# LIS-TU-Berlin/SVN-ICP

Measured on AMD Instinct MI355X. Metric: scan-pair registrations/sec at N particles x M source pts, 1/2/4/8 GPU, higher is better.
Workload: dtype f64; 1 GPU; C3: 128 particles SVN-ICP, 131072-pt source vs 262144-pt target, K=100, I=20, max_dist=1.0, lr=1.0, SVNFullGrad=False, correspondence=fast, early stop off; synthetic 64-beam scans (seed 20250718); particles=128, target_points=262144, knn_count=100, parallelism=single GPU

## Files before the change

### svn-icp_amd/csrc/api.hip

```cpp
#include "../../include/svnicp_hip.h"

#include <cmath>
#include <algorithm>
#include <cstdio>
#include <cstdlib>
#include <cstring>
#include <string>
#include <vector>

#include "device_buffer.hpp"
#include "information_solve.hpp"
#include "kernels.hpp"
#include "pose_prior.hpp"
#include "stage_a_host.hpp"
#include "stage_b_host.hpp"

using namespace svnicp;
using namespace svnicp_host;

namespace {

struct CloudState {
  DevBuf<double> src, tgt;
  bool src_set = false, tgt_set = false;
// ... 354 lines not shown
    HIPCHK(c, hipEventSynchronize(c->st.ev_init));
  }
  std::memcpy(c->st.h_init.p, init, (size_t)P * 48);
  HIPCHK(c, hipMemcpyAsync(c->st.init_pose.p, c->st.h_init.p, (size_t)P * 48, hipMemcpyHostToDevice, c->stream));
  HIPCHK(c, hipEventRecord(c->st.ev_init, c->stream));
  c->st.init_in_flight = true;
  c->st.host_stats_valid = false;
  const bool first = !c->run.particles_set || P != c->P;
  if (P != c->P) c->sc.have = false;
  c->sc.of_result = false;
  if (first && c->shard.row_world > 1) { c->shard.row_world = 1; c->shard.row_rank = 0; c->shard.B_total = 0; }
  c->P = P;
  if (!c->shard.set || first) { c->shard.p_lo = 0; c->shard.p_hi = P; c->shard.set = false; }
  HIPCHK(c, launch_init_particles(c->st.init_pose.p, P, c->pose0, c->prm.mode, c->st.R.p, c->st.t.p, c->st.Rtot.p, c->st.pose_out.p,
                                  (first || c->prm.mode == SVNICP_MODE_SVN) ? 1 : 0, c->st.eul.p, c->stream));
  c->run.particles_set = true;
  return SVNICP_OK;
}

int svnicp_set_initial_mean(svnicp_ctx* c, const double R0[9], const double t0[3]) {
  CTX_CHECK(c);
  if (!R0 || !t0) return fail(c, SVNICP_ERR_INVALID, "svnicp_set_initial_mean: null argument");
  std::memcpy(c->pose0.R0, R0, 9 * sizeof(double));
  std::memcpy(c->pose0.t0, t0, 3 * sizeof(double));
  c->run.have_candidates = false;
  return SVNICP_OK;
}

int svnicp_set_k(svnicp_ctx* c, int k) {
  CTX_CHECK(c);
  if (k < 1) return fail(c, SVNICP_ERR_INVALID, "svnicp_set_k: k >= 1 required");
  c->K = k;
  c->run.have_candidates = false;
  return SVNICP_OK;
}

int svnicp_set_max_dist(svnicp_ctx* c, double md) {
  CTX_CHECK(c);
  c->prm.max_dist = md;
  return SVNICP_OK;
}

int svnicp_set_option(svnicp_ctx* c, const char* name, const char* value) {
  CTX_CHECK(c);
  if (!name || !value) return fail(c, SVNICP_ERR_INVALID, "svnicp_set_option: null argument");
  const std::string k(name), v(value);
  Tuning& t = c->tune;
  auto num = [&](int lo, int hi, int* out) { char* end = nullptr; const long x = strtol(v.c_str(), &end, 10);
                                             if (end == v.c_str() || *end || x < lo || x > hi) return false; *out = (int)x; return true; };
  bool ok = true;
  if (k == "knn") { if (v == "auto") t.knn = {}; else if (v == "v1") t.knn = {false, KnnKernel::Stream}; else if (v == "v2") t.knn = {false, KnnKernel::SeededScan};
                    else if (v == "brute") t.knn = {false, KnnKernel::Brute}; else if (v == "tiles") t.knn = {false, KnnKernel::Tiles}; else ok = false; }
  else if (k == "knn_prefilter") { if (v == "mfma") t.knn_prefilter_mfma = 1; else if (v == "valu") t.knn_prefilter_mfma = 0; else ok = false; }
  else if (k == "fallback_sliced_max") ok = num(-1, 1 << 20, &t.fallback_sliced_max);
  else if (k == "accum") { if (v == "f64") t.accum = 0; else if (v == "valu") t.accum = 1; else if (v == "split") t.accum = 3; else ok = false; }
  else if (k == "update") { if (v == "auto") t.update_fused = 0; else if (v == "fused") t.update_fused = 1; else ok = false; }
  else if (k == "fused_update_max_p") ok = num(1, 700, &t.fused_update_max_p);
  else if (k == "wgpcu") { int x = 0, y = 0; ok = sscanf(v.c_str(), "%d,%d", &x, &y) == 2 && x >= 0 && x <= 64 && y >= 0 && y <= 16; if (ok) { t.wgpcu_search = x; t.wgpcu_accum = y; } }
  else if (k == "tp") ok = num(0, 1 << 16, &t.tp);
  else if (k == "debug") ok = num(0, 1, &t.debug);
  else if (k == "scan_split") ok = num(0, 16, &t.scan_split);
  else if (k == "group_stride") ok = num(0, 1 << 30, &t.group_stride);
  else if (k == "accum_min_steps") ok = num(0, 1 << 20, &t.accum_min_steps);
  else if (k == "brute_qb") { ok = num(0, 6, &t.brute_qb); }
  else if (k == "single") { if (v == "fused") t.single_fused = 1; else if (v == "split") t.single_fused = 0; else ok = false; }
  else if (k == "chain") { if (v == "auto") { t.small_chain = 1; t.persistent = 0; } else if (v == "persistent") { t.small_chain = 1; t.persistent = 1; }
                           else if (v == "general") { t.small_chain = 0; t.persistent = 0; } else ok = false; }
  else if (k == "median") { if (v == "auto") t.median_inline = -1; else if (v == "stream") t.median_inline = 0; else if (v == "inline") t.median_inline = 1; else ok = false; }
  else if (k == "sort") { if (v == "joint") t.sort_joint = 1; else if (v == "separate") t.sort_joint = 0; else ok = false; }
  else if (k == "sort_kernel") { if (v == "radix") t.sort_merge = 0; else if (v == "merge") t.sort_merge = 1; else ok = false; }
  else if (k == "table") { if (v == "select") t.table_select = 1; else if (v == "gather") t.table_select = 0; else ok = false; }
  else if (k == "correspondence") { if (v == "fast") t.full_corr = 0; else if (v == "full") t.full_corr = 1; else ok = false; }
  else return fail(c, SVNICP_ERR_INVALID, "svnicp_set_option: unknown option '" + k + "'");
  if (!ok) return fail(c, SVNICP_ERR_INVALID, "svnicp_set_option: bad value '" + v + "' for option '" + k + "'");
  c->run.have_candidates = false;
  c->sa.held = TargetLayout::None;
  if (c->run.began) c->st.step = plan_step(registration_facts(c, c->pl.on, c->pr.on), c->tune, c->sb.plan);
  return SVNICP_OK;
}

int svnicp_set_shard(svnicp_ctx* c, int p_lo, int p_hi) {
  CTX_CHECK(c);
  if (!c->run.particles_set || p_lo < 0 || p_hi > c->P || p_lo > p_hi)
    return fail(c, SVNICP_ERR_INVALID, "svnicp_set_shard: need 0 <= p_lo <= p_hi <= P after svnicp_set_particles");
  c->shard.p_lo = p_lo; c->shard.p_hi = p_hi; c->shard.set = true;
  return SVNICP_OK;
}

int svnicp_set_row_shard(svnicp_ctx* c, int row_rank, int row_world, int64_t total_source_points) {
  CTX_CHECK(c);
  if (!c->run.particles_set || row_world < 1 || row_rank < 0 || row_rank >= row_world || (row_world > 1 && total_source_points < 1))
    return fail(c, SVNICP_ERR_INVALID, "svnicp_set_row_shard: need 0 <= row_rank < row_world and the whole scan's point count, after svnicp_set_particles");
  if (bind(c)) return SVNICP_ERR_HIP;
  c->shard.row_rank = row_rank; c->shard.row_world = row_world;
  c->shard.B_total = row_world > 1 ? total_source_points : 0;
  if (row_world > 1) {
    HIPCHK(c, c->shard.rank_sums.ensure((size_t)row_world * c->P * kNSums));
    HIPCHK(c, hipMemsetAsync(c->shard.rank_sums.p, 0, (size_t)row_world * c->P * kNSums * sizeof(double), c->stream));
  }
  return SVNICP_OK;
}

void* svnicp_rank_sums_devptr(svnicp_ctx* c) { return (c && c->shard.row_world > 1) ? (void*)c->shard.rank_sums.p : nullptr; }

static bool normal_pass_due(const svnicp_ctx* c) {
  return c->pl.on && !c->pl.supplied && !(c->pl.estimated && c->pl.est_k == c->pl.normal_k);
// ... 1043 lines not shown
```

### svn-icp_amd/csrc/kernels.hpp

```cpp
#pragma once
#include "device_math.hpp"
#include "registration_plan.hpp"
#include "stage_a_plan.hpp"

namespace svnicp {

struct KnnArgs {
  const double* src;
  Pose0 pose;
  const double *tx, *ty, *tz;
  const int32_t* torig;
  int64_t M, Mp;
  int64_t b_lo, b_hi;
  int K, S;
  double* pool_d;
  int32_t* pool_i;
  int32_t* out_idx;
  double* out_d2;
  const int32_t* qlist;
  const int* qlist_count;
  int list_grid;
  int list_qw;
  int slices, slice_max_queries, merge_n;
  double* sl_d;
  int32_t* sl_i;
  const double* qthr;
};
hipError_t launch_knn_merge_slices(const KnnArgs& a, hipStream_t st);

struct KnnBruteArgs {
  const double* src;
  Pose0 pose;
  const double* tgt;
  int64_t M;
  int64_t b_lo, b_hi;
  int K;
  int32_t* out_idx;
  double* out_d2;
  unsigned long long* phase_cycles;
};
int knn_brute_queries_per_block(int64_t n, int num_cus);
hipError_t launch_knn_brute(const KnnBruteArgs& a, int num_cus, int queries_per_block, hipStream_t st);

struct KnnScanArgs {
  const double* src;
  Pose0 pose;
  const double *tx, *ty, *tz;
  const float *txf, *tyf, *tzf;
  const int32_t* torig;
  const unsigned long long* emax_bits;
  int64_t M, Mp, Ms;
  int64_t b_lo, b_hi;
  int K, S2, seed_rank;
  int32_t* pool;
  int32_t* out_idx;
  double* out_d2;
  int32_t* fail_list;
  int* fail_count;
};
hipError_t launch_targets_soa2(const double* tgt, int64_t M, int64_t Mp, double* tx, double* ty, double* tz,
                               float* txf, float* tyf, float* tzf, int32_t* torig, unsigned long long* emax_bits,
                               hipStream_t st);
hipError_t launch_knn_scan(const KnnScanArgs& a, hipStream_t st);
hipError_t launch_knn_topk(const KnnArgs& a, hipStream_t st);

struct KnnTilesArgs {
  const double* src;
  Pose0 pose;
  const int32_t* qorder;
  const double *tx, *ty, *tz;
  const float *txf, *tyf, *tzf;
  const int32_t* torig;
  const float* tile_box;
  const unsigned long long* emax_bits;
  const float4* tile_a;
  const float4* tile_o;
  int prefilter_mfma;
  int64_t M, Mp;
  int n_tiles;
  int64_t b_lo, b_hi;
  int K, S2;
  int32_t* pool;
  int32_t* arena;
  int32_t* chunk_tab;
  int arena_cap;
  int64_t tab_rows;
  int scan_split;
  unsigned int group_stride;
  int32_t* out_idx;
  double* out_d2;
  const double* tgt;
  float4* tbl_a;
  double* tbl_anchor;
  float* tbl_cmax;
  int32_t* fail_list;
  int* fail_count;
  int32_t* stat_n;
  unsigned long long* phase_cycles;
  void* qrec;
  double* fail_tau;
};
hipError_t launch_knn_tiles(const KnnTilesArgs& a, hipStream_t st);
hipError_t launch_candidate_dist2(const double* src, const Pose0& pose, const double* tgt, int64_t M, const int32_t* idx, int64_t B, int K,
                                  double* d2, hipStream_t st);
size_t sort_temp_bytes(size_t n, int key_bits);
hipError_t launch_bbox(const double* pts, int64_t n, unsigned long long* bbox, bool cleared, hipStream_t st);
hipError_t launch_morton_order(const double* pts, int64_t i0, int64_t n, int transform, const Pose0& pose,
                               const unsigned long long* bbox, unsigned int* keys_a, unsigned int* keys_b,
                               int32_t* vals_a, int32_t* order, void* temp, size_t temp_bytes, bool rocprim_sort, int32_t* fill_ff,
                               size_t fill_words, hipStream_t st);
hipError_t launch_morton_order_joint(const double* tgt, int64_t M, const double* qsrc, int64_t n, const Pose0& pose,
                                     const unsigned long long* bbox, unsigned int* keys_a, unsigned int* keys_b,
                                     int32_t* vals_a, int32_t* order, void* temp, size_t temp_bytes, bool rocprim_sort, int32_t* fill_ff,
                                     size_t fill_words, hipStream_t st);
hipError_t launch_targets_sorted(const double* tgt, int64_t M, int64_t Mp, const int32_t* order, double* tx, double* ty,
                                 double* tz, float* txf, float* tyf, float* tzf, int32_t* torig, float* tile_box,
                                 unsigned long long* emax_bits, bool emax_cleared, float4* tile_a, float4* tile_o, hipStream_t st);

struct AccumArgs {
  const double* src;
  const double* table;
  const float4* tablef;
  const float4* tablea;
  const float* cmax;
  int* ambig_count;
  const double* Rtot;
  int64_t B;
  int K, RS;
  int p_lo, p_hi;
  int TP;
// ... 200 lines not shown
```

### svn-icp_amd/csrc/knn_tiles.hip

```cpp
#include "kernels.hpp"
#include "stein_split_device.hpp"

namespace svnicp {

namespace {

constexpr int T = 8;
constexpr int STEP = kWave * T;
constexpr int QW = 64;
constexpr int WAVES = 4;
constexpr int QCAP = 1024;
constexpr int SL = 512;
constexpr int NSQ = 4;
constexpr int MAX_TILES = 8192;
constexpr int QB = 16;
constexpr double kU = 5.9604644775390625e-08;
constexpr float kEpsTile = 56.0f * 5.9604644775390625e-08f;

struct alignas(16) QF { float x, y, z, thr; };
struct alignas(16) QD { double x, y, z, tau; };

__device__ __forceinline__ void wave_sync() {
  __builtin_amdgcn_fence(__ATOMIC_ACQ_REL, "wavefront");
  __builtin_amdgcn_wave_barrier();
// ... 206 lines not shown
    return;
  }
  if (m <= 2 * kWave) {
    for (int e = m + lane; e < 2 * kWave + 8; e += kWave) { sd[e] = __builtin_huge_val(); si[e] = 0x7fffffff; }
    wave_sync();
    const int e0 = lane, e1 = lane + kWave;
    const double d0 = e0 < m ? sd[e0] : 0.0, d1 = e1 < m ? sd[e1] : 0.0;
    const int i0 = e0 < m ? si[e0] : 0, i1 = e1 < m ? si[e1] : 0;
    const P3 c0 = target_row(a, a.tbl_a && e0 < m, i0), c1 = target_row(a, a.tbl_a && e1 < m, i1);
    int* flag = si + 2 * kWave + 8;
    flag[lane] = 0; flag[lane + kWave] = 0;
    int r0 = 0, r1 = 0;
    for (int j0 = 0; j0 < m; j0 += 8) {
      double dj[8];
#pragma unroll
      for (int u = 0; u < 8; ++u) dj[u] = sd[j0 + u];
#pragma unroll
      for (int u = 0; u < 8; ++u) {
        r0 += dj[u] < d0 ? 1 : 0;
        r1 += dj[u] < d1 ? 1 : 0;
      }
    }
    wave_sync();
    if (e0 < m) atomicAdd(&flag[r0], 1);
    if (e1 < m) atomicAdd(&flag[r1], 1);
    wave_sync();
    if (__ballot((e0 < m && flag[r0] > 1) || (e1 < m && flag[r1] > 1))) {
      for (int j = 0; j < m; ++j) {
        const double dj = sd[j];
        const int ij = si[j];
        r0 += (dj == d0 && ij < i0) ? 1 : 0;
        r1 += (dj == d1 && ij < i1) ? 1 : 0;
      }
    }
    if (e0 < m && r0 < K) { a.out_idx[b * K + r0] = i0; if (a.out_d2) a.out_d2[b * K + r0] = d0; }
    if (e1 < m && r1 < K) { a.out_idx[b * K + r1] = i1; if (a.out_d2) a.out_d2[b * K + r1] = d1; }
    if (a.tbl_a) write_table_row(a, b, e0 < m ? r0 : -1, c0, e1 < m ? r1 : -1, c1, sd, lane);
    wave_sync();
  } else {
    int S = 256;
    while (S < m) S <<= 1;
    for (int e = m + lane; e < S; e += kWave) { sd[e] = __builtin_huge_val(); si[e] = 0x7fffffff; }
    wave_sync();
    bitonic_sort(sd, si, S, lane);
    for (int e = lane; e < K; e += kWave) { a.out_idx[b * K + e] = si[e]; if (a.out_d2) a.out_d2[b * K + e] = sd[e]; }
    if (a.tbl_a) {
      const int e1 = lane + kWave;
      write_table_row(a, b, lane, target_row(a, lane < K, si[lane]), e1, target_row(a, e1 < K, e1 < K ? si[e1] : 0), sd, lane);
    }
    wave_sync();
  }
}

__global__ __launch_bounds__(256) void k_knn_seed(KnnTilesArgs a) {
  extern __shared__ __align__(16) unsigned char smem[];
  const int lane = threadIdx.x & (kWave - 1);
  const int wave = __builtin_amdgcn_readfirstlane(threadIdx.x >> 6);
  const int K = a.K, n_tiles = a.n_tiles;
  constexpr size_t kShared = sizeof(QD) * QW + sizeof(QF) * QW + 4 * sizeof(int) * QW + sizeof(unsigned int) * (MAX_TILES / 32);
  constexpr size_t kScratch = sizeof(float2) * QB * kWave + 512;
  static_assert(QB * WAVES == QW, "one batch per wave");
  QD* qd = reinterpret_cast<QD*>(smem);
  QF* qf = reinterpret_cast<QF*>(smem + sizeof(QD) * QW);
  int* cnt = reinterpret_cast<int*>(smem + (sizeof(QD) + sizeof(QF)) * QW);
  int* qb = cnt + QW;
  float* thrb = reinterpret_cast<float*>(qb + QW);
  int* spare = reinterpret_cast<int*>(thrb + QW);
  unsigned int* tbits = reinterpret_cast<unsigned int*>(spare + QW);
  unsigned char* scratch = smem + kShared + kScratch * wave;
  float2* lm = reinterpret_cast<float2*>(scratch);

  const unsigned int grp = blockIdx.x;
  const int64_t q0 = a.b_lo + (int64_t)grp * QW;
  const int nq = (a.b_hi - q0) < QW ? (int)(a.b_hi - q0) : QW;
  const double Et = __longlong_as_double((long long)*a.emax_bits);

  unsigned long long tphase = a.phase_cycles ? __builtin_readcyclecounter() : 0ull;
  unsigned long long pacc[8] = {0, 0, 0, 0, 0, 0, 0, 0};
  auto phase_mark = [&](int i) {
    if (!a.phase_cycles) return;
    const unsigned long long now = __builtin_readcyclecounter();
    pacc[i] += now - tphase;
    tphase = now;
  };
  float wlo0 = 0.f, wlo1 = 0.f, wlo2 = 0.f, whi0 = 0.f, whi1 = 0.f, whi2 = 0.f;
  const int nwords = (n_tiles + 31) >> 5;
  if (wave == 0) {
    const bool act = lane < nq;
    const int64_t b = act ? (int64_t)a.qorder[q0 - a.b_lo + lane] : 0;
    QD s; s.x = s.y = s.z = 0.0; s.tau = 0.0;
    if (act) {
      stage_a_query(a.pose, a.src[3 * b], a.src[3 * b + 1], a.src[3 * b + 2], &s.x, &s.y, &s.z);
    }
    qd[lane] = s;
    QF f; f.x = (float)s.x; f.y = (float)s.y; f.z = (float)s.z; f.thr = -1.0f;
    qf[lane] = f;
    cnt[lane] = 0; qb[lane] = (int)b; thrb[lane] = -1.0f;
    const float inf = __builtin_huge_valf();
    wlo0 = act ? f32_floor(s.x) : inf; wlo1 = act ? f32_floor(s.y) : inf; wlo2 = act ? f32_floor(s.z) : inf;
    whi0 = act ? f32_ceil(s.x) : -inf; whi1 = act ? f32_ceil(s.y) : -inf; whi2 = act ? f32_ceil(s.z) : -inf;
    for (int off = 32; off > 0; off >>= 1) {
      wlo0 = __builtin_fminf(wlo0, __shfl_xor(wlo0, off, kWave)); whi0 = __builtin_fmaxf(whi0, __shfl_xor(whi0, off, kWave));
      wlo1 = __builtin_fminf(wlo1, __shfl_xor(wlo1, off, kWave)); whi1 = __builtin_fmaxf(whi1, __shfl_xor(whi1, off, kWave));
      wlo2 = __builtin_fminf(wlo2, __shfl_xor(wlo2, off, kWave)); whi2 = __builtin_fmaxf(whi2, __shfl_xor(whi2, off, kWave));
    }
  }
  wave_sync();
  const float* bx_lo0 = a.tile_box, *bx_lo1 = a.tile_box + n_tiles, *bx_lo2 = a.tile_box + 2 * (size_t)n_tiles;
  const float* bx_hi0 = a.tile_box + 3 * (size_t)n_tiles, *bx_hi1 = a.tile_box + 4 * (size_t)n_tiles,
             * bx_hi2 = a.tile_box + 5 * (size_t)n_tiles;

  {
    if (wave == 0) {
      for (int e = lane; e < nwords; e += kWave) tbits[e] = 0u;
      wave_sync();
      const float px = qf[lane].x, py = qf[lane].y, pz = qf[lane].z;
      unsigned long long best[NSQ];
#pragma unroll
      for (int i = 0; i < NSQ; ++i) best[i] = ~0ull;
      float4* boxs = reinterpret_cast<float4*>(scratch);
      const int n_groups = (n_tiles + kWave - 1) / kWave;
      unsigned int gkey[2] = {0xffffffffu, 0xffffffffu};
      for (int g = 0; g < n_groups; ++g) {
        const int tl = g * kWave + lane;
        const float inf = __builtin_huge_valf();
        float lo0 = inf, lo1 = inf, lo2 = inf, hi0 = -inf, hi1 = -inf, hi2 = -inf;
        if (tl < n_tiles) { lo0 = bx_lo0[tl]; lo1 = bx_lo1[tl]; lo2 = bx_lo2[tl]; hi0 = bx_hi0[tl]; hi1 = bx_hi1[tl]; hi2 = bx_hi2[tl]; }
        for (int off = 32; off > 0; off >>= 1) {
          lo0 = __builtin_fminf(lo0, __shfl_xor(lo0, off, kWave)); hi0 = __builtin_fmaxf(hi0, __shfl_xor(hi0, off, kWave));
          lo1 = __builtin_fminf(lo1, __shfl_xor(lo1, off, kWave)); hi1 = __builtin_fmaxf(hi1, __shfl_xor(hi1, off, kWave));
          lo2 = __builtin_fminf(lo2, __shfl_xor(lo2, off, kWave)); hi2 = __builtin_fmaxf(hi2, __shfl_xor(hi2, off, kWave));
        }
        const float glb = box_lb2(wlo0, wlo1, wlo2, whi0, whi1, whi2, lo0, lo1, lo2, hi0, hi1, hi2);
        const unsigned int key = (glb < inf) ? ((__float_as_uint(glb) & ~127u) | (unsigned int)g) : 0xffffffffu;
        if (lane == (g & (kWave - 1))) gkey[g >> 6] = key;
      }
      for (;;) {
        unsigned int kmin = gkey[0] < gkey[1] ? gkey[0] : gkey[1];
        for (int off = 32; off > 0; off >>= 1) { const unsigned int o = __shfl_xor(kmin, off, kWave); kmin = o < kmin ? o : kmin; }
        if (kmin == 0xffffffffu) break;
        float w4 = -__builtin_huge_valf();
        if (lane < nq) w4 = best[NSQ - 1] == ~0ull ? __builtin_huge_valf() : __uint_as_float((unsigned int)(best[NSQ - 1] >> 32));
        for (int off = 32; off > 0; off >>= 1) w4 = __builtin_fmaxf(w4, __shfl_xor(w4, off, kWave));
        if (__uint_as_float(kmin & ~127u) > w4) break;
        const int gsel = (int)(kmin & 127u);
        if (lane == (gsel & (kWave - 1))) gkey[gsel >> 6] = 0xffffffffu;
        const int t0 = gsel * kWave;
        const int tl = t0 + lane;
        if (tl < n_tiles) {
          boxs[2 * lane] = make_float4(bx_lo0[tl], bx_lo1[tl], bx_lo2[tl], bx_hi0[tl]);
          boxs[2 * lane + 1] = make_float4(bx_hi1[tl], bx_hi2[tl], 0.f, 0.f);
        }
        wave_sync();
        const int cntt = (n_tiles - t0) < kWave ? (n_tiles - t0) : kWave;
#pragma unroll 4
        for (int i = 0; i < cntt; ++i) {
          const float4 b0 = boxs[2 * i], b1 = boxs[2 * i + 1];
          const float l0 = b0.x, l1 = b0.y, l2 = b0.z, h0 = b0.w, h1 = b1.x, h2 = b1.y;
          const int tile = t0 + i;
          const float lb = box_lb2(px, py, pz, px, py, pz, l0, l1, l2, h0, h1, h2);
          const float c0 = px - 0.5f * (l0 + h0), c1 = py - 0.5f * (l1 + h1), c2 = pz - 0.5f * (l2 + h2);
          const float score = lb + 1e-3f * (c0 * c0 + c1 * c1 + c2 * c2);
          unsigned long long key = (score < __builtin_huge_valf()) ? (((unsigned long long)__float_as_uint(score) << 32) | (unsigned int)tile) : ~0ull;
#pragma unroll
          for (int u = 0; u < NSQ; ++u) {
            const unsigned long long lo = key < best[u] ? key : best[u];
            key = key < best[u] ? best[u] : key;
            best[u] = lo;
          }
        }
        wave_sync();
      }
      if (lane < nq) {
#pragma unroll
        for (int i = 0; i < NSQ; ++i)
          if (best[i] != ~0ull) { const unsigned int t = (unsigned int)(best[i] & 0xffffffffull); atomicOr(&tbits[t >> 5], 1u << (t & 31)); }
      }
    }
    phase_mark(0);
    __syncthreads();
    phase_mark(3);
    const int qb0 = wave * QB;
    if (qb0 < nq) {
      const int nb = (nq - qb0) < QB ? (nq - qb0) : QB;
      for (int e = lane; e < QB * kWave; e += kWave) lm[e] = make_float2(__builtin_huge_valf(), __builtin_huge_valf());
      wave_sync();
      for (int wd = 0; wd < nwords; ++wd) {
        unsigned int bits = __builtin_amdgcn_readfirstlane(tbits[wd]);
        while (bits) {
          const int tile = (wd << 5) + (int)__builtin_ctz(bits);
          bits &= bits - 1;
          if (a.phase_cycles) pacc[4] += 1;
          const int64_t tb = (int64_t)tile * STEP;
          float x[T], y[T], z[T];
#pragma unroll
          for (int t = 0; t < T; ++t) { x[t] = a.txf[tb + t * kWave + lane]; y[t] = a.tyf[tb + t * kWave + lane]; z[t] = a.tzf[tb + t * kWave + lane]; }
          for (int q = 0; q < nb; ++q) {
            const float4 cur = *reinterpret_cast<const float4*>(&qf[qb0 + q]);
            float2 m = lm[q * kWave + lane];
#pragma unroll
            for (int t = 0; t < T; ++t) {
              const float dx = cur.x - x[t], dy = cur.y - y[t], dz = cur.z - z[t];
              float d = __builtin_fmaf(dz, dz, __builtin_fmaf(dy, dy, dx * dx));
              d = __builtin_fminf(d, __builtin_huge_valf());
              m.y = __builtin_amdgcn_fmed3f(m.x, m.y, d);
              m.x = __builtin_fminf(m.x, d);
            }
            lm[q * kWave + lane] = m;
          }
        }
      }
      wave_sync();
      phase_mark(5);
      for (int q = 0; q < nb; ++q) {
        const float2 m = lm[q * kWave + lane];
        const unsigned int kx = __float_as_uint(m.x), ky = __float_as_uint(m.y);
        unsigned int kth = 0u;
        for (int bit = 30; bit >= 0; --bit) {
          const unsigned int t_try = kth | ((1u << bit) - 1u);
          const int c = __popcll(__ballot(kx <= t_try)) + __popcll(__ballot(ky <= t_try));
          if (c < K) kth |= 1u << bit;
        }
        if (lane == 0) spare[qb0 + q] = (int)kth;
      }
      phase_mark(6);
    }
    phase_mark(1);
    __syncthreads();
    phase_mark(3);
    if (wave == 0 && lane < nq) {
      const double tv = (double)__uint_as_float((unsigned int)spare[lane]);
      const double E = fmax(Et, fmax(fabs(qd[lane].x), fmax(fabs(qd[lane].y), fabs(qd[lane].z))));
      double tau = __builtin_huge_val();
      if (tv < (double)__builtin_huge_valf()) {
        const double r = sqrt(tv) * (1.0 + 1e-6) + 4.0 * kU * E;
        tau = (r * r) * (1.0 + 1e-12);
      }
      qd[lane].tau = tau;
      const float thr = filter_threshold(tau, E);
      qf[lane].thr = thr;
      float tb = __builtin_huge_valf();
      if (thr < __builtin_huge_valf()) {
        const double rb = sqrt((double)thr) + 2.0 * kU * E;
        tb = f32_round_up((rb * rb) * (1.0 + 1e-6));
      }
      thrb[lane] = tb;
    }
    wave_sync();
  }

  if (wave == 0 && lane < nq) {
    QRec rec;
    rec.x = qd[lane].x; rec.y = qd[lane].y; rec.z = qd[lane].z; rec.tau = qd[lane].tau;
    rec.cnt = 0; rec.row = qb[lane]; rec.thr = qf[lane].thr; rec.tb = thrb[lane];
    reinterpret_cast<QRec*>(a.qrec)[q0 + lane] = rec;
  }
  phase_mark(1);
  if (a.phase_cycles && lane == 0) {
#pragma unroll
    for (int i = 0; i < 5; ++i) atomicAdd(&a.phase_cycles[i], pacc[i]);
    unsigned long long* pw = a.phase_cycles + 8 + 8 * ((size_t)grp * WAVES + wave);
#pragma unroll
    for (int i = 0; i < 7; ++i) pw[i] = pacc[i];
  }
}

template <int SW, bool MF>
__global__ __launch_bounds__(64 * SW) __attribute__((amdgpu_waves_per_eu(4, 4))) void k_knn_scan_tiles(KnnTilesArgs a) {
  __shared__ __align__(16) QF s_qf[QW];
  __shared__ int s_cnt[QW];
  __shared__ int s_ticket;
  __shared__ __align__(16) int2 s_queue[SW][QCAP];
  __shared__ __align__(16) float4 s_lb[MF ? SW : 1][QW];
  __shared__ float s_lth[MF ? SW : 1][QW];
  __shared__ int s_lq[MF ? SW : 1][QW];
  const int lane = threadIdx.x & (kWave - 1);
  const int wave = __builtin_amdgcn_readfirstlane(threadIdx.x >> 6);
  const int S2 = a.S2, n_tiles = a.n_tiles;
  int2* queue = s_queue[wave];
  const unsigned int ngrp = gridDim.x;
  const unsigned int grp = (unsigned int)(((unsigned long long)blockIdx.x * a.group_stride) % ngrp);
  const int64_t q0 = a.b_lo + (int64_t)grp * QW;
  const int nq = (a.b_hi - q0) < QW ? (int)(a.b_hi - q0) : QW;
  QRec* recs = reinterpret_cast<QRec*>(a.qrec);
  unsigned long long tphase = a.phase_cycles ? __builtin_readcyclecounter() : 0ull;
  unsigned long long pacc[8] = {0, 0, 0, 0, 0, 0, 0, 0};
  auto phase_mark = [&](int i) {
    if (!a.phase_cycles) return;
    const unsigned long long now = __builtin_readcyclecounter();
    pacc[i] += now - tphase;
    tphase = now;
  };
  float gx = 0.f, gy = 0.f, gz = 0.f, gtb = -1.0f, gthr = -1.0f;
  float wlo0, wlo1, wlo2, whi0, whi1, whi2, tmax;
  {
    const bool act = lane < nq;
    QF f; f.x = f.y = f.z = 0.f; f.thr = -1.0f;
    const float inf = __builtin_huge_valf();
    wlo0 = wlo1 = wlo2 = inf; whi0 = whi1 = whi2 = -inf;
    if (act) {
      const QRec rec = recs[q0 + lane];
      f.x = (float)rec.x; f.y = (float)rec.y; f.z = (float)rec.z; f.thr = rec.thr;
      gtb = rec.tb; gthr = rec.thr;
      wlo0 = f32_floor(rec.x); wlo1 = f32_floor(rec.y); wlo2 = f32_floor(rec.z);
      whi0 = f32_ceil(rec.x); whi1 = f32_ceil(rec.y); whi2 = f32_ceil(rec.z);
    }
    gx = f.x; gy = f.y; gz = f.z;
    if (wave == 0) { s_qf[lane] = f; s_cnt[lane] = 0; }
    if (threadIdx.x == 0) s_ticket = 0;
    tmax = gtb;
    for (int off = 32; off > 0; off >>= 1) {
      wlo0 = __builtin_fminf(wlo0, __shfl_xor(wlo0, off, kWave)); whi0 = __builtin_fmaxf(whi0, __shfl_xor(whi0, off, kWave));
      wlo1 = __builtin_fminf(wlo1, __shfl_xor(wlo1, off, kWave)); whi1 = __builtin_fmaxf(whi1, __shfl_xor(whi1, off, kWave));
      wlo2 = __builtin_fminf(wlo2, __shfl_xor(wlo2, off, kWave)); whi2 = __builtin_fmaxf(whi2, __shfl_xor(whi2, off, kWave));
      tmax = __builtin_fmaxf(tmax, __shfl_xor(tmax, off, kWave));
    }
// ... 232 lines not shown
  __shared__ int s_si[WAVES][SL];
  const int lane = threadIdx.x & (kWave - 1);
  const int wave = __builtin_amdgcn_readfirstlane(threadIdx.x >> 6);
  const QRec* recs = reinterpret_cast<const QRec*>(a.qrec);
  for (int64_t r = a.b_lo + (int64_t)blockIdx.x * WAVES + wave; r < a.b_hi; r += (int64_t)gridDim.x * WAVES) {
    const QRec rec = recs[r];
    select_query(a, r, rec, s_sd[wave], s_si[wave], lane);
  }
}

__global__ __launch_bounds__(256) void k_candidate_dist2(const double* __restrict__ src, Pose0 pose, const double* __restrict__ tgt, int64_t M,
                                                         const int32_t* __restrict__ idx, int64_t B, int K, double* __restrict__ d2) {
  const int lane = threadIdx.x & (kWave - 1);
  const int wave = __builtin_amdgcn_readfirstlane(threadIdx.x >> 6);
  for (int64_t b = (int64_t)blockIdx.x * WAVES + wave; b < B; b += (int64_t)gridDim.x * WAVES) {
    double qx, qy, qz;
    stage_a_query(pose, src[3 * b], src[3 * b + 1], src[3 * b + 2], &qx, &qy, &qz);
    int first0 = 0x7fffffff;
    for (int k0 = 0; k0 < K && first0 == 0x7fffffff; k0 += kWave) {
      const unsigned long long z = __ballot(k0 + lane < K && idx[b * K + k0 + lane] == 0);
      if (z) first0 = k0 + (int)__builtin_ctzll(z);
    }
    for (int k = lane; k < K; k += kWave) {
      int64_t i = idx[b * K + k];
      const bool pad = i == 0 && k > first0;
      i = i < 0 ? 0 : (i >= M ? M - 1 : i);
      const double dx = qx - tgt[3 * i], dy = qy - tgt[3 * i + 1], dz = qz - tgt[3 * i + 2];
      const double d = (dx * dx + dy * dy) + dz * dz;
      d2[b * K + k] = (pad || d != d) ? 0.0 : d;
    }
  }
}

}

hipError_t launch_candidate_dist2(const double* src, const Pose0& pose, const double* tgt, int64_t M, const int32_t* idx, int64_t B, int K,
                                  double* d2, hipStream_t st) {
  if (B <= 0 || K <= 0) return hipSuccess;
  int64_t nb = (B + WAVES - 1) / WAVES;
  if (nb > 65536) nb = 65536;
  hipLaunchKernelGGL(k_candidate_dist2, dim3((unsigned)nb), dim3(256), 0, st, src, pose, tgt, M, idx, B, K, d2);
  return hipGetLastError();
}

static_assert(STEP == kTileSlots && MAX_TILES == kMaxTiles, "knn_tiles_applicable (stage_a_plan.hpp) speaks of this kernel's tiles");

hipError_t launch_knn_tiles(const KnnTilesArgs& a, hipStream_t st) {
  const int64_t nq = a.b_hi - a.b_lo;
  if (nq <= 0) return hipSuccess;
  const int64_t nb = (nq + QW - 1) / QW;
  if (a.n_tiles > MAX_TILES) return hipErrorInvalidValue;
  const size_t smem = sizeof(QD) * QW + sizeof(QF) * QW + 4 * sizeof(int) * QW + sizeof(unsigned int) * (MAX_TILES / 32) +
                      (sizeof(float2) * QB * kWave + 512) * WAVES;
  hipError_t e = hipFuncSetAttribute(reinterpret_cast<const void*>(k_knn_seed),
                                     hipFuncAttributeMaxDynamicSharedMemorySize, (int)smem);
  if (e != hipSuccess) return e;
  hipLaunchKernelGGL(k_knn_seed, dim3((unsigned)nb), dim3(256), smem, st, a);
  e = hipGetLastError();
  if (e != hipSuccess) return e;
  const dim3 sgrid((unsigned)((nq + QW - 1) / QW));
  if (a.prefilter_mfma) {
    if (a.scan_split == 4) hipLaunchKernelGGL((k_knn_scan_tiles<4, true>), sgrid, dim3(256), 0, st, a);
    else hipLaunchKernelGGL((k_knn_scan_tiles<8, true>), sgrid, dim3(512), 0, st, a);
  } else {
    if (a.scan_split == 4) hipLaunchKernelGGL((k_knn_scan_tiles<4, false>), sgrid, dim3(256), 0, st, a);
    else hipLaunchKernelGGL((k_knn_scan_tiles<8, false>), sgrid, dim3(512), 0, st, a);
  }
  e = hipGetLastError();
  if (e != hipSuccess) return e;
  int64_t nbs = (nq + WAVES - 1) / WAVES;
  if (nbs > 65536) nbs = 65536;
  hipLaunchKernelGGL(k_knn_select, dim3((unsigned)nbs), dim3(256), 0, st, a);
  return hipGetLastError();
}

}
```

### svn-icp_amd/csrc/registration_plan.hpp

```cpp
#pragma once
#include <cstddef>
#include <cstdint>
#include <initializer_list>

#include "stage_a_plan.hpp"

namespace svnicp {

struct Tuning {
  KnnOption knn;
  int knn_prefilter_mfma = 1;
  int fallback_sliced_max = -1;
  int accum = 3;
  int update_fused = 0;
  int fused_update_max_p = 128;
  int wgpcu_search = 0, wgpcu_accum = 0;
  int tp = 0;
  int accum_min_steps = 0;
  int group_stride = 0;
  int scan_split = 0;
  int debug = 0;
  int single_fused = 1;
  int small_chain = 1;
  int persistent = 0;
  int median_inline = -1;
  int brute_qb = 0;
  int sort_joint = 1;
  int sort_merge = 0;
  int table_select = 1;
  int full_corr = 0;
};

struct RegistrationFacts {
  int P = 0, K = 0, I = 0;
  int64_t B = 0, M = 0;
  bool svgd = false, check_early_stop = false, record_trace = false;
  bool profiling = false;
  bool shard_set = false;
  int p_lo = 0, p_hi = 0;
  int row_world = 1;
  int batch = 0;
  bool explicit_tab = false;
  int tab_I = 0;
  bool plane = false;
  bool normals_supplied = false;
  int normal_k = 16;
  int weighting = 0;
  bool prior = false;
  int nshard() const { return p_hi - p_lo; }
  bool whole_shard() const { return p_lo == 0 && p_hi == P; }
};

constexpr int64_t kMinibatchMaxRows = 1ll << 22;
struct RegistrationRows {
  bool mb;
  int64_t Bq;
  int64_t Bt;
  int64_t Bi;
};
inline RegistrationRows registration_rows(int batch, int I, int64_t B) {
  if (batch == 0 || I <= 0) return {false, B, B, B};
  const int64_t n = (int64_t)I * batch;
  return {true, B < n ? B : n, n, batch};
}
// ... 170 lines not shown
```

### svn-icp_amd/csrc/stage_a_host.hpp

```cpp
#pragma once
#include <algorithm>
#include <cstdio>
#include <initializer_list>
#include <vector>

#include "device_buffer.hpp"
#include "kernels.hpp"

namespace svnicp_host {
using namespace svnicp;

struct StageAEnv {
  hipStream_t stream;
  const Tuning& tune;
  int num_cus;
  bool record_trace;
  const double* tgt;
  int64_t B, M;
  const Pose0& pose0;
};

struct TableOut { float4* rows; double* anchor; float* cmax; };

struct StageA {
// ... 79 lines not shown
    return ensure_layout(o, e);
  }

  template <class Obj>
  int ensure_layout(Obj* o, const StageAEnv& e) {
    layout_pending = false;
    start_words_set = false;
    if (held == plan.layout || plan.layout == TargetLayout::None) return SVNICP_OK;
    if (plan.layout == TargetLayout::Hashed) {
      HIPCHK(o, launch_targets_soa2(e.tgt, e.M, plan.Mp, tx.p, ty.p, tz.p, txf.p, tyf.p, tzf.p, torig.p, emax.p, e.stream));
    } else {
      HIPCHK(o, launch_bbox(e.tgt, e.M, bbox.p, false, e.stream));
      HIPCHK(o, launch_morton_order(e.tgt, 0, e.M, 0, e.pose0, bbox.p, keys_a.p, keys_b.p, vals_a.p, order_t.p, sort_tmp.p, sort_tmp_bytes,
                                    e.tune.sort_merge != 0, nullptr, 0, e.stream));
      HIPCHK(o, launch_targets_sorted(e.tgt, e.M, plan.Mp, order_t.p, tx.p, ty.p, tz.p, txf.p, tyf.p, tzf.p, torig.p, tile_box.p, emax.p, false, tile_a.p, tile_o.p, e.stream));
    }
    held = plan.layout;
    return SVNICP_OK;
  }

  hipError_t launch_fallback(KnnArgs a, hipStream_t stream) {
    a.qlist = fail_list.p; a.qlist_count = fail_count.p; a.list_grid = kFallbackGrid; a.list_qw = kFallbackQW;
    a.slice_max_queries = plan.sliced_max; a.slices = 0;
    hipError_t e = launch_knn_topk(a, stream);
    if (e != hipSuccess || plan.sliced_max <= 0) return e;
    a.slices = knn_slice_count(a.K);
    a.merge_n = 1;
    while (a.merge_n < a.slices * a.K) a.merge_n <<= 1;
    a.sl_d = sl_d.p; a.sl_i = sl_i.p;
    e = launch_knn_topk(a, stream);
    if (e != hipSuccess) return e;
    return launch_knn_merge_slices(a, stream);
  }

  template <class Obj>
  int clear_dbg_phase(Obj* o, hipStream_t stream, size_t waves) {
    HIPCHK(o, dbg_phase.ensure(8 + 8 * kDbgPhaseWaves));
    HIPCHK(o, hipMemsetAsync(dbg_phase.p, 0, (8 + 8 * waves) * sizeof(unsigned long long), stream));
    return SVNICP_OK;
  }

  template <class Obj>
  int print_phases(Obj* o, const StageAEnv& e, int64_t n, size_t dbg_waves) {
    std::vector<unsigned long long> h(8 + 8 * dbg_waves);
    HIPCHK(o, hipMemcpyAsync(h.data(), dbg_phase.p, h.size() * sizeof(unsigned long long), hipMemcpyDeviceToHost, e.stream));
    HIPCHK(o, hipStreamSynchronize(e.stream));
    if (plan.kernel == KnnKernel::Brute) {
      const int qb = e.tune.brute_qb > 0 ? e.tune.brute_qb : knn_brute_queries_per_block(n, e.num_cus);
      const double nwg = (double)((n + qb - 1) / qb);
      fprintf(stderr, "[svnicp] k_knn_brute (%d queries per workgroup) thread-0 cycles per workgroup: pass A %.0f, bound %.0f, pass B %.0f, general path %.0f, rank + write %.0f\n",
              qb, h[0] / nwg, h[1] / nwg, h[2] / nwg, h[3] / nwg, h[4] / nwg);
      return SVNICP_OK;
    }
    fprintf(stderr, "[svnicp] k_knn_tiles wave cycles: rank %llu seed %llu scan %llu barrier waits + hand-over %llu | counts: seed tiles %llu scan tiles %llu scan (query, tile) pairs %llu\n", h[0], h[1], h[2], h[3], h[4], h[5], h[6]);
    auto column = [&](const char* tag, int col, unsigned long long floor_) {
      std::vector<unsigned long long> v;
      for (size_t w = 0; w < dbg_waves; ++w) { const unsigned long long x = h[8 + 8 * w + col]; if (x >= floor_) v.push_back(x); }
      if (v.empty()) return;
      std::sort(v.begin(), v.end());
      fprintf(stderr, "[svnicp]   seed kernel %-12s n %6zu  p50 %8llu  p90 %8llu  p99 %8llu  max %8llu cycles\n", tag, v.size(), v[v.size() / 2],
              v[v.size() * 9 / 10], v[v.size() * 99 / 100], v.back());
    };
    column("rank", 0, 5000); column("seed", 1, 1); column("tile loop", 5, 1); column("bisection", 6, 1); column("waits", 3, 0);
    return SVNICP_OK;
  }

  template <class Obj>
  int search(Obj* o, const StageAEnv& e, const double* qsrc, const Pose0& pose, int K, int32_t* out_idx, double* out_d2, int64_t b_lo,
             int64_t b_hi, const TableOut* tbl = nullptr, bool whole_source = false) {
    const int64_t n = b_hi - b_lo;
    const bool joint = layout_pending && whole_source && plan.kernel == KnnKernel::Tiles && b_lo == 0 && n == e.B && n > 0;
    if (layout_pending && !joint)
      if (const int rc = ensure_layout(o, e)) return rc;
    const bool words_set = start_words_set && joint;
    start_words_set = false;
    KnnArgs a{};
    a.src = qsrc; a.pose = pose; a.tx = tx.p; a.ty = ty.p; a.tz = tz.p; a.torig = torig.p;
    a.M = e.M; a.Mp = plan.Mp; a.b_lo = b_lo; a.b_hi = b_hi; a.K = K; a.S = knn_pool_size(K);
    a.pool_d = pool_d.p; a.pool_i = pool_i.p; a.out_idx = out_idx; a.out_d2 = out_d2;
    switch (plan.kernel) {
    case KnnKernel::Brute: {
      KnnBruteArgs k{};
      k.src = qsrc; k.pose = pose; k.tgt = e.tgt; k.M = e.M; k.b_lo = b_lo; k.b_hi = b_hi; k.K = K; k.out_idx = out_idx; k.out_d2 = out_d2;
      if (e.tune.debug) {
        if (const int rc = clear_dbg_phase(o, e.stream, 0)) return rc;
        k.phase_cycles = dbg_phase.p;
      }
      HIPCHK(o, launch_knn_brute(k, e.num_cus, e.tune.brute_qb, e.stream));
      if (e.tune.debug) return print_phases(o, e, n, 0);
      return SVNICP_OK;
    }
    case KnnKernel::Tiles: {
      if (n <= 0) return SVNICP_OK;
      const int32_t* qord = qorder.p + b_lo;
      const size_t tab_words = tiles_chunk_tab_words(plan.rows);
      if (joint) {
        HIPCHK(o, launch_bbox(e.tgt, e.M, bbox.p, words_set, e.stream));
        HIPCHK(o, launch_morton_order_joint(e.tgt, e.M, qsrc, n, pose, bbox.p, keys_a.p, keys_b.p, vals_a.p, order_t.p, sort_tmp.p, sort_tmp_bytes,
                                            e.tune.sort_merge != 0, chunk_tab.p, tab_words, e.stream));
        HIPCHK(o, launch_targets_sorted(e.tgt, e.M, plan.Mp, order_t.p, tx.p, ty.p, tz.p, txf.p, tyf.p, tzf.p, torig.p, tile_box.p, emax.p, words_set, tile_a.p, tile_o.p, e.stream));
        held = plan.layout; layout_pending = false;
        qord = order_t.p + e.M;
      } else {
        HIPCHK(o, launch_morton_order(qsrc, b_lo, n, 1, pose, bbox.p, keys_a.p, keys_b.p, vals_a.p, qorder.p + b_lo, sort_tmp.p, sort_tmp_bytes,
                                      e.tune.sort_merge != 0, chunk_tab.p, tab_words, e.stream));
      }
      KnnTilesArgs k{};
      k.src = qsrc; k.pose = pose; k.qorder = qord;
      k.tx = tx.p; k.ty = ty.p; k.tz = tz.p; k.txf = txf.p; k.tyf = tyf.p; k.tzf = tzf.p;
      k.torig = torig.p; k.tile_box = tile_box.p; k.emax_bits = emax.p;
      k.tile_a = tile_a.p; k.tile_o = tile_o.p; k.prefilter_mfma = e.tune.knn_prefilter_mfma;
      k.M = e.M; k.Mp = plan.Mp; k.n_tiles = (int)(plan.Mp / kTileSlots); k.b_lo = b_lo; k.b_hi = b_hi; k.K = K; k.S2 = plan.S2;
      k.pool = pool2.p; k.out_idx = out_idx; k.out_d2 = tbl ? nullptr : out_d2;
      k.tgt = e.tgt;
      if (tbl) { k.tbl_a = tbl->rows; k.tbl_anchor = tbl->anchor; k.tbl_cmax = tbl->cmax; }
      k.arena = arena.p; k.chunk_tab = chunk_tab.p; k.arena_cap = plan.arena_cap; k.tab_rows = plan.rows;
      k.scan_split = e.tune.scan_split == 4 ? 4 : 8;
      {
        const unsigned int ng = (unsigned int)((n + 63) / 64);
        unsigned int st = e.tune.group_stride > 0 ? (unsigned int)e.tune.group_stride : 17u;
        auto gcd = [](unsigned int x, unsigned int y) { while (y) { const unsigned int t = x % y; x = y; y = t; } return x; };
        while (st > 1 && gcd(st, ng) != 1) st += 2;
        if (ng <= 2 || st >= ng) st = 1;
        k.group_stride = st;
      }
      k.fail_list = fail_list.p; k.fail_count = fail_count.p; k.fail_tau = fail_tau.p; k.qrec = qrec.p;
      a.qthr = fail_tau.p;
      if (e.record_trace) k.stat_n = stat_n.p;
      if (!words_set) HIPCHK(o, hipMemsetAsync(fail_count.p, 0, sizeof(int), e.stream));
      const size_t dbg_waves = (size_t)((n + 63) / 64) * 4;
      const bool dbg = e.tune.debug && dbg_waves <= kDbgPhaseWaves;
      if (dbg) {
        if (const int rc = clear_dbg_phase(o, e.stream, dbg_waves)) return rc;
        k.phase_cycles = dbg_phase.p;
      }
      HIPCHK(o, launch_knn_tiles(k, e.stream));
      if (dbg)
        if (const int rc = print_phases(o, e, n, dbg_waves)) return rc;
      HIPCHK(o, launch_fallback(a, e.stream));
      if (tbl)
        HIPCHK(o, launch_build_table3_list(out_idx, fail_list.p, fail_count.p, e.B, K, e.tgt, e.M, tbl->anchor, tbl->rows, tbl->cmax, e.stream));
      return SVNICP_OK;
    }
    case KnnKernel::SeededScan: {
      KnnScanArgs k{};
      k.src = qsrc; k.pose = pose; k.tx = tx.p; k.ty = ty.p; k.tz = tz.p;
      k.txf = txf.p; k.tyf = tyf.p; k.tzf = tzf.p; k.torig = torig.p; k.emax_bits = emax.p;
      k.M = e.M; k.Mp = plan.Mp; k.Ms = plan.scan_Ms; k.b_lo = b_lo; k.b_hi = b_hi; k.K = K; k.S2 = plan.S2;
      k.seed_rank = plan.scan_rank; k.pool = pool2.p; k.out_idx = out_idx; k.out_d2 = out_d2;
      k.fail_list = fail_list.p; k.fail_count = fail_count.p;
      HIPCHK(o, hipMemsetAsync(fail_count.p, 0, sizeof(int), e.stream));
      HIPCHK(o, launch_knn_scan(k, e.stream));
      HIPCHK(o, launch_fallback(a, e.stream));
      return SVNICP_OK;
    }
    case KnnKernel::Stream:
      HIPCHK(o, launch_knn_topk(a, e.stream));
    }
    return SVNICP_OK;
  }

  int64_t block_rows(int64_t n) const { return std::max<int64_t>(1, std::min<int64_t>(plan.rows, n)); }
  template <class Obj, class Done = int (*)(int64_t, int64_t)>
  int search_blocks(Obj* o, const StageAEnv& e, const double* q, int64_t n, int Kq, int32_t* out_idx, double* out_d2, int out_step,
// ... 31 lines not shown
```

Measured before the change: 151.3 registrations/s.

## Bound seed-tile ranking by per-tile lower bounds and parallelize group box reduction

In the KNN seed kernel's rank phase, each tile in a selected group now gets a wave-level lower bound. The wave bitonic-sorts those bounds and scores only tiles that could still beat the current fourth-best, stopping early once sorted. The group bounding-box reduction is rewritten so several groups are reduced per pass with a smaller shuffle tree, and the ranking wave gets raised scheduling priority. A full-ranking template path stays available through a new option, and a counter of scored tiles is added to the debug trace.

```diff
diff --git a/svn-icp_amd/csrc/api.hip b/svn-icp_amd/csrc/api.hip
--- a/svn-icp_amd/csrc/api.hip
+++ b/svn-icp_amd/csrc/api.hip
@@ -430,6 +430,7 @@
   if (k == "knn") { if (v == "auto") t.knn = {}; else if (v == "v1") t.knn = {false, KnnKernel::Stream}; else if (v == "v2") t.knn = {false, KnnKernel::SeededScan};
                     else if (v == "brute") t.knn = {false, KnnKernel::Brute}; else if (v == "tiles") t.knn = {false, KnnKernel::Tiles}; else ok = false; }
   else if (k == "knn_prefilter") { if (v == "mfma") t.knn_prefilter_mfma = 1; else if (v == "valu") t.knn_prefilter_mfma = 0; else ok = false; }
+  else if (k == "seed_rank") { if (v == "bounded") t.seed_rank_full = 0; else if (v == "full") t.seed_rank_full = 1; else ok = false; }
   else if (k == "fallback_sliced_max") ok = num(-1, 1 << 20, &t.fallback_sliced_max);
   else if (k == "accum") { if (v == "f64") t.accum = 0; else if (v == "valu") t.accum = 1; else if (v == "split") t.accum = 3; else ok = false; }
   else if (k == "update") { if (v == "auto") t.update_fused = 0; else if (v == "fused") t.update_fused = 1; else ok = false; }
diff --git a/svn-icp_amd/csrc/kernels.hpp b/svn-icp_amd/csrc/kernels.hpp
--- a/svn-icp_amd/csrc/kernels.hpp
+++ b/svn-icp_amd/csrc/kernels.hpp
@@ -76,6 +76,7 @@
   const float4* tile_a;
   const float4* tile_o;
   int prefilter_mfma;
+  int seed_rank_full;
   int64_t M, Mp;
   int n_tiles;
   int64_t b_lo, b_hi;
diff --git a/svn-icp_amd/csrc/knn_tiles.hip b/svn-icp_amd/csrc/knn_tiles.hip
--- a/svn-icp_amd/csrc/knn_tiles.hip
+++ b/svn-icp_amd/csrc/knn_tiles.hip
@@ -282,6 +282,7 @@
   }
 }
 
+template <bool BOUNDED>
 __global__ __launch_bounds__(256) void k_knn_seed(KnnTilesArgs a) {
   extern __shared__ __align__(16) unsigned char smem[];
   const int lane = threadIdx.x & (kWave - 1);
@@ -342,6 +343,7 @@
 
   {
     if (wave == 0) {
+      __builtin_amdgcn_s_setprio(2);
       for (int e = lane; e < nwords; e += kWave) tbits[e] = 0u;
       wave_sync();
       const float px = qf[lane].x, py = qf[lane].y, pz = qf[lane].z;
@@ -351,20 +353,51 @@
       float4* boxs = reinterpret_cast<float4*>(scratch);
       const int n_groups = (n_tiles + kWave - 1) / kWave;
       unsigned int gkey[2] = {0xffffffffu, 0xffffffffu};
-      for (int g = 0; g < n_groups; ++g) {
-        const int tl = g * kWave + lane;
-        const float inf = __builtin_huge_valf();
-        float lo0 = inf, lo1 = inf, lo2 = inf, hi0 = -inf, hi1 = -inf, hi2 = -inf;
-        if (tl < n_tiles) { lo0 = bx_lo0[tl]; lo1 = bx_lo1[tl]; lo2 = bx_lo2[tl]; hi0 = bx_hi0[tl]; hi1 = bx_hi1[tl]; hi2 = bx_hi2[tl]; }
-        for (int off = 32; off > 0; off >>= 1) {
-          lo0 = __builtin_fminf(lo0, __shfl_xor(lo0, off, kWave)); hi0 = __builtin_fmaxf(hi0, __shfl_xor(hi0, off, kWave));
-          lo1 = __builtin_fminf(lo1, __shfl_xor(lo1, off, kWave)); hi1 = __builtin_fmaxf(hi1, __shfl_xor(hi1, off, kWave));
-          lo2 = __builtin_fminf(lo2, __shfl_xor(lo2, off, kWave)); hi2 = __builtin_fmaxf(hi2, __shfl_xor(hi2, off, kWave));
-        }
-        const float glb = box_lb2(wlo0, wlo1, wlo2, whi0, whi1, whi2, lo0, lo1, lo2, hi0, hi1, hi2);
-        const unsigned int key = (glb < inf) ? ((__float_as_uint(glb) & ~127u) | (unsigned int)g) : 0xffffffffu;
-        if (lane == (g & (kWave - 1))) gkey[g >> 6] = key;
-      }
+      {
+        unsigned int* gk = reinterpret_cast<unsigned int*>(scratch + sizeof(float4) * 2 * kWave);
+        int lgp = 3;
+        while (lgp < 6 && (n_groups << (lgp + 1)) <= kWave) ++lgp;
+        const int GP = 1 << lgp, sub = lane & (GP - 1), gpb = kWave >> lgp;
+        for (int g0 = 0; g0 < n_groups; g0 += gpb) {
+          const int g = g0 + (lane >> lgp);
+          const float inf = __builtin_huge_valf();
+          float lo0 = inf, lo1 = inf, lo2 = inf, hi0 = -inf, hi1 = -inf, hi2 = -inf;
+          if (g < n_groups) {
+#pragma unroll 8
+            for (int i = sub; i < kWave; i += GP) {
+              const int tl = g * kWave + i;
+              if (tl < n_tiles) {
+                lo0 = __builtin_fminf(lo0, bx_lo0[tl]); lo1 = __builtin_fminf(lo1, bx_lo1[tl]); lo2 = __builtin_fminf(lo2, bx_lo2[tl]);
+                hi0 = __builtin_fmaxf(hi0, bx_hi0[tl]); hi1 = __builtin_fmaxf(hi1, bx_hi1[tl]); hi2 = __builtin_fmaxf(hi2, bx_hi2[tl]);
+              }
+            }
+          }
+          for (int off = GP >> 1; off > 0; off >>= 1) {
+            lo0 = __builtin_fminf(lo0, __shfl_xor(lo0, off, kWave)); hi0 = __builtin_fmaxf(hi0, __shfl_xor(hi0, off, kWave));
+            lo1 = __builtin_fminf(lo1, __shfl_xor(lo1, off, kWave)); hi1 = __builtin_fmaxf(hi1, __shfl_xor(hi1, off, kWave));
+            lo2 = __builtin_fminf(lo2, __shfl_xor(lo2, off, kWave)); hi2 = __builtin_fmaxf(hi2, __shfl_xor(hi2, off, kWave));
+          }
+          const float glb = box_lb2(wlo0, wlo1, wlo2, whi0, whi1, whi2, lo0, lo1, lo2, hi0, hi1, hi2);
+          if (sub == 0 && g < n_groups) gk[g] = (glb < inf) ? ((__float_as_uint(glb) & ~127u) | (unsigned int)g) : 0xffffffffu;
+        }
+        wave_sync();
+        if (lane < n_groups) gkey[0] = gk[lane];
+        if (lane + kWave < n_groups) gkey[1] = gk[lane + kWave];
+      }
+      auto score_tile = [&](int i, int tile) {
+        const float4 b0 = boxs[2 * i], b1 = boxs[2 * i + 1];
+        const float l0 = b0.x, l1 = b0.y, l2 = b0.z, h0 = b0.w, h1 = b1.x, h2 = b1.y;
+        const float lb = box_lb2(px, py, pz, px, py, pz, l0, l1, l2, h0, h1, h2);
+        const float c0 = px - 0.5f * (l0 + h0), c1 = py - 0.5f * (l1 + h1), c2 = pz - 0.5f * (l2 + h2);
+        const float score = lb + 1e-3f * (c0 * c0 + c1 * c1 + c2 * c2);
+        unsigned long long key = (score < __builtin_huge_valf()) ? (((unsigned long long)__float_as_uint(score) << 32) | (unsigned int)tile) : ~0ull;
+#pragma unroll
+        for (int u = 0; u < NSQ; ++u) {
+          const unsigned long long lo = key < best[u] ? key : best[u];
+          key = key < best[u] ? best[u] : key;
+          best[u] = lo;
+        }
+      };
       for (;;) {
         unsigned int kmin = gkey[0] < gkey[1] ? gkey[0] : gkey[1];
         for (int off = 32; off > 0; off >>= 1) { const unsigned int o = __shfl_xor(kmin, off, kWave); kmin = o < kmin ? o : kmin; }
@@ -377,27 +410,51 @@
         if (lane == (gsel & (kWave - 1))) gkey[gsel >> 6] = 0xffffffffu;
         const int t0 = gsel * kWave;
         const int tl = t0 + lane;
+        unsigned int tkey = 0xffffffffu;
         if (tl < n_tiles) {
-          boxs[2 * lane] = make_float4(bx_lo0[tl], bx_lo1[tl], bx_lo2[tl], bx_hi0[tl]);
-          boxs[2 * lane + 1] = make_float4(bx_hi1[tl], bx_hi2[tl], 0.f, 0.f);
+          const float l0 = bx_lo0[tl], l1 = bx_lo1[tl], l2 = bx_lo2[tl], h0 = bx_hi0[tl], h1 = bx_hi1[tl], h2 = bx_hi2[tl];
+          boxs[2 * lane] = make_float4(l0, l1, l2, h0);
+          boxs[2 * lane + 1] = make_float4(h1, h2, 0.f, 0.f);
+          if constexpr (BOUNDED) {
+            const float lbt = box_lb2(wlo0, wlo1, wlo2, whi0, whi1, whi2, l0, l1, l2, h0, h1, h2);
+            if (lbt < __builtin_huge_valf()) tkey = (__float_as_uint(lbt) & ~63u) | (unsigned int)lane;
+          }
         }
         wave_sync();
-        const int cntt = (n_tiles - t0) < kWave ? (n_tiles - t0) : kWave;
+        if constexpr (BOUNDED) {
+          auto passes = [&]() { return __ballot(tkey != 0xffffffffu && __uint_as_float(tkey & ~63u) <= w4); };
+          unsigned long long todo = passes();
+          const bool sorted = __popcll(todo) > 4;
+          if (sorted) {
+#pragma unroll
+            for (int k = 2; k <= kWave; k <<= 1)
+#pragma unroll
+              for (int j = k >> 1; j > 0; j >>= 1) {
+                const unsigned int o = (unsigned int)__shfl_xor((int)tkey, j, kWave);
+                const bool keep_min = ((lane & k) == 0) == ((lane & j) == 0);
+                const unsigned int mn = o < tkey ? o : tkey, mx = o < tkey ? tkey : o;
+                tkey = keep_min ? mn : mx;
+              }
+            todo = passes();
+          }
+          while (todo) {
+            const int i = (int)__builtin_ctzll(todo);
+            todo &= todo - 1;
+            const unsigned int k = (unsigned int)__builtin_amdgcn_readlane((int)tkey, i);
+            const float lbt = __uint_as_float(k & ~63u);
+            const float b4 = __uint_as_float((unsigned int)(best[NSQ - 1] >> 32));
+            if (!__ballot(lane < nq && !(b4 < lbt))) {
+              if (sorted) break;
+              continue;
+            }
+            if (a.phase_cycles) pacc[7] += 1;
+            score_tile((int)(k & 63u), t0 + (int)(k & 63u));
+          }
+        } else {
+          const int cntt = (n_tiles - t0) < kWave ? (n_tiles - t0) : kWave;
+          if (a.phase_cycles) pacc[7] += cntt;
 #pragma unroll 4
-        for (int i = 0; i < cntt; ++i) {
-          const float4 b0 = boxs[2 * i], b1 = boxs[2 * i + 1];
-          const float l0 = b0.x, l1 = b0.y, l2 = b0.z, h0 = b0.w, h1 = b1.x, h2 = b1.y;
-          const int tile = t0 + i;
-          const float lb = box_lb2(px, py, pz, px, py, pz, l0, l1, l2, h0, h1, h2);
-          const float c0 = px - 0.5f * (l0 + h0), c1 = py - 0.5f * (l1 + h1), c2 = pz - 0.5f * (l2 + h2);
-          const float score = lb + 1e-3f * (c0 * c0 + c1 * c1 + c2 * c2);
-          unsigned long long key = (score < __builtin_huge_valf()) ? (((unsigned long long)__float_as_uint(score) << 32) | (unsigned int)tile) : ~0ull;
-#pragma unroll
-          for (int u = 0; u < NSQ; ++u) {
-            const unsigned long long lo = key < best[u] ? key : best[u];
-            key = key < best[u] ? best[u] : key;
-            best[u] = lo;
-          }
+          for (int i = 0; i < cntt; ++i) score_tile(i, t0 + i);
         }
         wave_sync();
       }
@@ -406,6 +463,7 @@
         for (int i = 0; i < NSQ; ++i)
           if (best[i] != ~0ull) { const unsigned int t = (unsigned int)(best[i] & 0xffffffffull); atomicOr(&tbits[t >> 5], 1u << (t & 31)); }
       }
+      __builtin_amdgcn_s_setprio(0);
     }
     phase_mark(0);
     __syncthreads();
@@ -491,7 +549,7 @@
     for (int i = 0; i < 5; ++i) atomicAdd(&a.phase_cycles[i], pacc[i]);
     unsigned long long* pw = a.phase_cycles + 8 + 8 * ((size_t)grp * WAVES + wave);
 #pragma unroll
-    for (int i = 0; i < 7; ++i) pw[i] = pacc[i];
+    for (int i = 0; i < 8; ++i) pw[i] = pacc[i];
   }
 }
 
@@ -830,10 +888,10 @@
   if (a.n_tiles > MAX_TILES) return hipErrorInvalidValue;
   const size_t smem = sizeof(QD) * QW + sizeof(QF) * QW + 4 * sizeof(int) * QW + sizeof(unsigned int) * (MAX_TILES / 32) +
                       (sizeof(float2) * QB * kWave + 512) * WAVES;
-  hipError_t e = hipFuncSetAttribute(reinterpret_cast<const void*>(k_knn_seed),
-                                     hipFuncAttributeMaxDynamicSharedMemorySize, (int)smem);
+  auto seed = a.seed_rank_full ? k_knn_seed<false> : k_knn_seed<true>;
+  hipError_t e = hipFuncSetAttribute(reinterpret_cast<const void*>(seed), hipFuncAttributeMaxDynamicSharedMemorySize, (int)smem);
   if (e != hipSuccess) return e;
-  hipLaunchKernelGGL(k_knn_seed, dim3((unsigned)nb), dim3(256), smem, st, a);
+  hipLaunchKernelGGL(seed, dim3((unsigned)nb), dim3(256), smem, st, a);
   e = hipGetLastError();
   if (e != hipSuccess) return e;
   const dim3 sgrid((unsigned)((nq + QW - 1) / QW));
diff --git a/svn-icp_amd/csrc/registration_plan.hpp b/svn-icp_amd/csrc/registration_plan.hpp
--- a/svn-icp_amd/csrc/registration_plan.hpp
+++ b/svn-icp_amd/csrc/registration_plan.hpp
@@ -10,6 +10,7 @@
 struct Tuning {
   KnnOption knn;
   int knn_prefilter_mfma = 1;
+  int seed_rank_full = 0;
   int fallback_sliced_max = -1;
   int accum = 3;
   int update_fused = 0;
diff --git a/svn-icp_amd/csrc/stage_a_host.hpp b/svn-icp_amd/csrc/stage_a_host.hpp
--- a/svn-icp_amd/csrc/stage_a_host.hpp
+++ b/svn-icp_amd/csrc/stage_a_host.hpp
@@ -155,7 +155,9 @@
               qb, h[0] / nwg, h[1] / nwg, h[2] / nwg, h[3] / nwg, h[4] / nwg);
       return SVNICP_OK;
     }
-    fprintf(stderr, "[svnicp] k_knn_tiles wave cycles: rank %llu seed %llu scan %llu barrier waits + hand-over %llu | counts: seed tiles %llu scan tiles %llu scan (query, tile) pairs %llu\n", h[0], h[1], h[2], h[3], h[4], h[5], h[6]);
+    unsigned long long ranked = 0;
+    for (size_t w = 0; w < dbg_waves; ++w) ranked += h[8 + 8 * w + 7];
+    fprintf(stderr, "[svnicp] k_knn_tiles wave cycles: rank %llu seed %llu scan %llu barrier waits + hand-over %llu | counts: rank tiles scored %llu seed tiles %llu scan tiles %llu scan (query, tile) pairs %llu\n", h[0], h[1], h[2], h[3], ranked, h[4], h[5], h[6]);
     auto column = [&](const char* tag, int col, unsigned long long floor_) {
       std::vector<unsigned long long> v;
       for (size_t w = 0; w < dbg_waves; ++w) { const unsigned long long x = h[8 + 8 * w + col]; if (x >= floor_) v.push_back(x); }
@@ -212,7 +214,7 @@
       k.src = qsrc; k.pose = pose; k.qorder = qord;
       k.tx = tx.p; k.ty = ty.p; k.tz = tz.p; k.txf = txf.p; k.tyf = tyf.p; k.tzf = tzf.p;
       k.torig = torig.p; k.tile_box = tile_box.p; k.emax_bits = emax.p;
-      k.tile_a = tile_a.p; k.tile_o = tile_o.p; k.prefilter_mfma = e.tune.knn_prefilter_mfma;
+      k.tile_a = tile_a.p; k.tile_o = tile_o.p; k.prefilter_mfma = e.tune.knn_prefilter_mfma; k.seed_rank_full = e.tune.seed_rank_full;
       k.M = e.M; k.Mp = plan.Mp; k.n_tiles = (int)(plan.Mp / kTileSlots); k.b_lo = b_lo; k.b_hi = b_hi; k.K = K; k.S2 = plan.S2;
       k.pool = pool2.p; k.out_idx = out_idx; k.out_d2 = tbl ? nullptr : out_d2;
       k.tgt = e.tgt;
```

New measurement: 153.1 registrations/s (median of 6 runs). 1.01x the previous value.
